# ska-sa/katsdpsigproc

Measured on AMD Instinct MI355X. Metric: visibility samples/s (baselines x channels) through full RFI flagger, higher is better.
Workload: dtype f32 amplitude / f64 deviations

## Files before the change

### katsdpsigproc_amd/csrc/ring_kernel.h

```cpp
#pragma once
#include "fused_common.h"

#ifndef RING_STOP
#define RING_STOP 0
#endif
#define RING_THREADS 512
#define RING_STRIP 8
#define RING_NSLOT 32
#ifndef RING_G
#define RING_G 4
#endif
#ifndef RING_PRIO
#define RING_PRIO 0
#endif
#ifndef RING_STAGGER
#define RING_STAGGER 0
#endif
#define RING_SLOT_BYTES 4096
#define RING_LIST_DOUBLES 256
#define RING_XCD_GROUP 8

struct RingLayout {
    static constexpr size_t RING_BYTES = (size_t)RING_NSLOT * RING_SLOT_BYTES;
    static constexpr size_t LIST_BYTES = sizeof(double) * RING_LIST_DOUBLES * RING_STRIP;
    static constexpr size_t CTRL_BYTES = 64;
    static constexpr size_t LDS_BYTES = RING_BYTES + LIST_BYTES + CTRL_BYTES;
};

#ifdef RING_TRACE
#define RING_TRACE_STRIPS 24
#define RING_TRACE_SLOTS 16
__device__ unsigned long long ring_trace_buf[256 * 8 * RING_TRACE_STRIPS * RING_TRACE_SLOTS];
#endif

#define RING_WORK_LIST 2
#define RING_WORK_DONE 10

__device__ __forceinline__ int ring_strip_of(int x, int t)
{
    return ((t / RING_XCD_GROUP) * 8 + x) * RING_XCD_GROUP + (t % RING_XCD_GROUP);
}

__device__ __forceinline__ int ring_take(unsigned *work, int x, int n_strips, int t0)
{
    for (int k = 0; k < 8; k++) {
        const int xx = (x + k) & 7;
        const int t = t0 + (int)atomicAdd(&work[RING_WORK_LIST + xx], 1u);
        const int s = ring_strip_of(xx, t);
        if (s < n_strips) return s;
    }
    return -1;
}

__device__ __forceinline__ float ring_from_next(float v, float edge, int lane)
{
    const float r = __shfl_down(v, 1, 64);
    return lane == 63 ? edge : r;
}
__device__ __forceinline__ float ring_from_prev(float v, float edge, int lane)
{
    const float r = __shfl_up(v, 1, 64);
    return lane == 0 ? edge : r;
}

template <int WIDTH>
__global__ __launch_bounds__(RING_THREADS) void flagger_ring_kernel(const FusedParams p)
{
    constexpr int R = 64, W = WIDTH, H = WIDTH / 2;
    constexpr int G = RING_G, NSLOT = RING_NSLOT, STEPS = 64, NCHUNK = STEPS / G;
    constexpr int K = NSLOT / G;
    constexpr int PER_CHUNK = G / 2;
    static_assert(W % 2 == 1 && W <= 13 && 2 * H <= G * 3, "merging median only");
    typedef __attribute__((address_space(3))) void lds_void;
    extern __shared__ __attribute__((aligned(16))) char lds[];
    const int tid = threadIdx.x, lane = tid & 63;
    const int wave = __builtin_amdgcn_readfirstlane(tid >> 6);
    const int C = p.channels;
    double *list = (double *)(lds + RingLayout::RING_BYTES) + wave * RING_LIST_DOUBLES;
    int *ctrl = (int *)(lds + RingLayout::RING_BYTES + RingLayout::LIST_BYTES);
    const unsigned lds_base = (unsigned)(size_t)(lds_void *)lds;

    const int q = wave & 3, par = wave >> 2;
    const int rl = lane >> 2;
    const int chunk16 = (lane & 3) ^ ((rl >> 2) & 3);
    const size_t row_bytes = (size_t)p.vis_stride * 8;
    const unsigned lane_off = (unsigned)((size_t)(16 * q + rl) * 64 * row_bytes + (size_t)chunk16 * 16);
    const int pp = wave >> 1, hh = wave & 1;
    const int l16 = lane & 15;
    const unsigned rd_off = (lane >> 4) * 1024 + l16 * 64 + ((pp ^ ((l16 >> 2) & 3)) * 16) + 8 * hh;
    typedef const __attribute__((address_space(3))) char lds_cchar;
    typedef const __attribute__((address_space(3))) unsigned long long lds_cu64;
    lds_cchar *lds3 = (lds_cchar *)(lds_void *)lds;

    unsigned long long run_src = 0;
    const unsigned long long rb2 = 2 * (unsigned long long)row_bytes;
    const unsigned piece_base = __builtin_amdgcn_readfirstlane(lds_base + q * 1024);
    auto issue = [&](int slot) {
        unsigned pb = piece_base;
        asm volatile("" : "+s"(pb));
        const unsigned dst = pb + (unsigned)(slot + par) * RING_SLOT_BYTES;
        unsigned keep;
        asm volatile("s_mov_b32 %0, m0\n\ts_mov_b32 m0, %3\n\ts_nop 0\n\t"
                     "global_load_lds_dwordx4 %1, %2\n\ts_mov_b32 m0, %0"
                     : "=&s"(keep) : "v"(lane_off), "s"(run_src), "s"(dst) : "memory");
        run_src += rb2;
    };
    auto strip_base = [&](int strip) -> const char * {
        return (const char *)p.vis + (size_t)strip * (RING_STRIP * 8);
    };

    const int xcd = blockIdx.x & 7;
    const int per_list = (int)gridDim.x >> 3;
    const int t0 = p.n_static * per_list;
    auto static_strip = [&](int k) { return ring_strip_of(xcd, k * per_list + ((int)blockIdx.x >> 3)); };
    if (tid == 0) {
        int s0 = 0 < p.n_static ? static_strip(0) : ring_take(p.work, xcd, p.n_strips, t0);
        int s1 = -1;
        if (s0 >= 0) s1 = 1 < p.n_static ? static_strip(1) : ring_take(p.work, xcd, p.n_strips, t0);
        ctrl[0] = s0;
        ctrl[1] = s1;
    }
    __syncthreads();
    int cur = __builtin_amdgcn_readfirstlane(ctrl[0]), nxt = __builtin_amdgcn_readfirstlane(ctrl[1]);
    int k_strip = 0;
    auto finish = [&]() {
        if (tid == 0 && atomicAdd(&p.work[RING_WORK_DONE], 1u) == gridDim.x - 1u) {
#pragma unroll
            for (int k = RING_WORK_LIST; k <= RING_WORK_DONE; k++) p.work[k] = 0;
        }
    };
    if (cur < 0) {
        finish();
        return;
    }
#if RING_STAGGER > 0
    if ((blockIdx.x >> 3) & 1) {
#pragma unroll
        for (int i = 0; i < RING_STAGGER; i++) __builtin_amdgcn_s_sleep(127);
    }
#endif
    auto start_of = [&](int strip) -> unsigned long long {
        const unsigned long long a = (unsigned long long)strip_base(strip) + (unsigned long long)par * row_bytes;
        return ((unsigned long long)(unsigned)__builtin_amdgcn_readfirstlane((unsigned)(a >> 32)) << 32) |
               (unsigned long long)(unsigned)__builtin_amdgcn_readfirstlane((unsigned)a);
    };
    run_src = start_of(cur);
#pragma unroll
    for (int j = 0; j < NSLOT; j += 2) issue(j);
    float2 zz[2][G];
    {
        constexpr int AH0 = (K - 1) * PER_CHUNK;
        __builtin_amdgcn_s_waitcnt(0x0070 | (AH0 & 15) | ((AH0 >> 4) << 14));
        __syncthreads();
#pragma unroll
        for (int g = 0; g < G; g++) {
            const unsigned long long w = *(lds_cu64 *)(lds3 + rd_off + g * RING_SLOT_BYTES);
            zz[0][g] = make_float2(__uint_as_float((unsigned)w), __uint_as_float((unsigned)(w >> 32)));
        }
    }
    const float nanv = __builtin_nanf("");
    const float2 *visf = (const float2 *)p.vis;

#if RING_PRIO == 1
    if (wave >= 4) __builtin_amdgcn_s_setprio(1);
#endif
    int mad_hint = -1;
    const int lane_id = lane;
#ifdef RING_TRACE
    int trace_it = 0;
#define RING_STAMP(i)                                                                              \
    do {                                                                                           \
        if (lane_id == 0 && trace_it < RING_TRACE_STRIPS && blockIdx.x < 256)                      \
            ring_trace_buf[((blockIdx.x * 8 + wave) * RING_TRACE_STRIPS + trace_it) * RING_TRACE_SLOTS + (i)] =   \
                __builtin_amdgcn_s_memtime();                                                      \
    } while (0)
#else
#define RING_STAMP(i) do { } while (0)
#endif
    for (;;) {
        int lane = lane_id;
        asm volatile("" : "+v"(lane));
        const int bl = cur * RING_STRIP + wave;
        const bool more = nxt >= 0;
        const unsigned long long start_nxt = start_of(more ? nxt : cur);
        auto fetch = [&](int c) -> float {
            const bool inside = c >= 0 && c < C;
            const int cc = inside ? c : 0;
            const float2 v = visf[(size_t)cc * p.vis_stride + bl];
            float a = ksp_abs_c64(v.x, v.y);
            return inside ? a : nanv;
        };
        RING_STAMP(0);
#ifdef RING_TRACE
        unsigned long long wait_dma = 0, wait_bar = 0;
        if (lane_id == 0 && trace_it < RING_TRACE_STRIPS && blockIdx.x < 256)
            ring_trace_buf[((blockIdx.x * 8 + wave) * RING_TRACE_STRIPS + trace_it) * RING_TRACE_SLOTS + 4] = __builtin_amdgcn_s_memrealtime();
#endif
        float amp[STEPS];
        unsigned umax = 0;
        auto load_chunk = [&](auto c_) {
            constexpr int c = decltype(c_)::value;
            constexpr int AH = (K - 2) * PER_CHUNK;
#ifdef RING_TRACE
            unsigned long long w0;
            asm volatile("s_memtime %0\n\ts_waitcnt lgkmcnt(0)" : "=s"(w0));
#endif
            if (more || (c + K - 1) * G + G <= STEPS)
                __builtin_amdgcn_s_waitcnt(0x0070 | (AH & 15) | ((AH >> 4) << 14));
            else
                __builtin_amdgcn_s_waitcnt(0x0070);
#ifdef RING_TRACE
            unsigned long long w1;
            asm volatile("s_memtime %0\n\ts_waitcnt lgkmcnt(0)" : "=s"(w1));
#endif
#ifndef RING_NOSYNC
            __syncthreads();
#endif
#ifdef RING_TRACE
            unsigned long long w2;
            asm volatile("s_memtime %0\n\ts_waitcnt lgkmcnt(0)" : "=s"(w2));
            wait_dma += w1 - w0;
            wait_bar += w2 - w1;
#endif
            ksp_static_for<G / 2>([&](auto u_) {
                constexpr int j = c * G + 2 * decltype(u_)::value + NSLOT;
                if constexpr (j < STEPS) {
                    issue(j % NSLOT);
                } else if (more) {
                    if constexpr (j == STEPS) run_src = start_nxt;
                    issue(j % NSLOT);
                }
            });
            if (c + 1 < NCHUNK || more) {
                unsigned ro = rd_off + (((c + 1) * G) % NSLOT) * RING_SLOT_BYTES;
                asm volatile("" : "+v"(ro));
#pragma unroll
                for (int g = 0; g < G; g++) {
                    const unsigned long long w = *(lds_cu64 *)(lds3 + ro + g * RING_SLOT_BYTES);
                    zz[(c + 1) & 1][g] = make_float2(__uint_as_float((unsigned)w), __uint_as_float((unsigned)(w >> 32)));
                }
            }
#if RING_PRIO == 2
            if ((c + (wave >> 2)) & 1)
                __builtin_amdgcn_s_setprio(1);
            else
                __builtin_amdgcn_s_setprio(0);
#endif
            const float2 (&z)[G] = zz[c & 1];
            unsigned key = ~0u;
#pragma unroll
            for (int g = 0; g < G; g++) key &= ksp_abs_range_key(z[g].x, z[g].y);
#pragma unroll
            for (int g = 0; g < G; g += 2)
                ksp_abs_c64_inrange_x2(z[g].x, z[g].y, z[g + 1].x, z[g + 1].y, amp[c * G + g],
                                       amp[c * G + g + 1]);
            if (ksp_any((key & KSP_ABS_RANGE_BIT) == 0)) {
#pragma unroll
                for (int g = 0; g < G; g++) {
                    amp[c * G + g] = ksp_abs_c64(z[g].x, z[g].y);
                    umax = max(umax, __float_as_uint(amp[c * G + g]));
                }
            }
        };

        float dev[R];
        float dmax;
        unsigned ex_a = 0, ex_b = 0;
        int tiny = 0;
        auto note_exact = [&](unsigned &acc, float x, float m, float d) {
            unsigned t;
            asm("v_min_u32 %1, %2, %3\n\tv_or_b32 %1, 0x7fffff, %1\n\t"
                "v_cmp_ge_f32 vcc, %1, |%4|\n\tv_addc_co_u32 %0, vcc, %0, %0, vcc"
                : "+v"(acc), "=&v"(t)
                : "v"(__float_as_uint(x)), "v"(__float_as_uint(m)), "v"(d)
                : "vcc");
        };
#if RING_STOP == 1
        dmax = 0.f;
        ksp_static_for<NCHUNK>([&](auto c_) {
            load_chunk(c_);
            constexpr int c = decltype(c_)::value;
#pragma unroll
            for (int g = 0; g < G; g++) {
                dev[c * G + g] = amp[c * G + g];
                dmax += amp[c * G + g];
            }
        });
#else
        {
            MergeMedian<R, W> mm;
            mm.pinf = __builtin_inff();
            mm.ninf = -__builtin_inff();
            asm volatile("" : "+v"(mm.pinf), "+v"(mm.ninf));
            const float pinf = mm.pinf, ninf = mm.ninf;
            const bool first = lane == 0, last = lane == 63;
            dmax = ninf;
            float rh[H];
            auto X = [&](auto i_) -> float {
                constexpr int i = decltype(i_)::value;
                if constexpr (i < STEPS) {
                    if constexpr (i % G == 0) load_chunk(std::integral_constant<int, i / G>{});
                    return amp[i];
                } else {
                    if constexpr (i == STEPS) {
#pragma unroll
                        for (int k = 0; k < H; k++)
                            rh[k] = ring_from_next(amp[k], (k & 1) ? ninf : pinf, lane);
                    }
                    return rh[i - STEPS];
                }
            };
            constexpr int RV = R - H;
            constexpr int STAGES = (RV + W - 1) / W;
            using MM = MergeMedian<R, W>;
            float cur_b[W];
            ksp_static_for<W>([&](auto k_) { cur_b[decltype(k_)::value] = X(k_); });
            ksp_static_for<STAGES>([&](auto m_) {
                constexpr int m = decltype(m_)::value;
                float S[MM::S_SIZE];
                S[MM::off(W - 1)] = cur_b[W - 1];
                ksp_static_for<W - 1>([&](auto u_) {
                    constexpr int t = W - 2 - decltype(u_)::value;
                    mm.template insert<W - 1 - t>(&S[MM::off(t + 1)], cur_b[t], &S[MM::off(t)]);
                });
                float P[W], nxt_b[W];
                ksp_static_for<W>([&](auto t_) {
                    constexpr int t = decltype(t_)::value;
                    constexpr int jv = m * W + t;
                    if constexpr (jv < RV) {
                        constexpr int j = jv + H;
                        if constexpr (t >= 1) {
                            nxt_b[t - 1] = X(std::integral_constant<int, (m + 1) * W + t - 1>{});
                            if constexpr (t == 1)
                                P[0] = nxt_b[0];
                            else
                                mm.template insert<t - 1>(P, nxt_b[t - 1], P);
                        }
                        const float med = mm.template rank<W - t, t, H>(&S[MM::off(t)], P);
                        const float xc = (t + H < W) ? cur_b[t + H < W ? t + H : 0] : nxt_b[t + H >= W ? t + H - W : 0];
                        float d = xc - med;
                        constexpr bool right_odd = j + H >= R && ((j + H - R + 1) & 1);
                        if constexpr (right_odd) {
                            const float lo = mm.template rank<W - t, t, H - 1>(&S[MM::off(t)], P);
                            if (last) {
                                const double dd = (double)xc - ((double)lo + (double)med) * 0.5;
                                d = (float)dd;
                                tiny += (d == 0.0f && dd != 0.0);
                            }
                        }
                        asm volatile("" : "+v"(d));
                        if constexpr (jv < 32)
                            note_exact(ex_a, xc, med, d);
                        else
                            note_exact(ex_b, xc, med, d);
                        if constexpr (jv & 1)
                            asm("v_max3_f32 %0, %0, %1, %2" : "+v"(dmax) : "v"(dev[j - 1]), "v"(d));
                        else if constexpr (jv == RV - 1)
                            dmax = mm.vmax(dmax, d);
                        dev[j] = d;
                    }
                });
                if constexpr (m + 1 < STAGES) {
                    ksp_static_for<W>([&](auto k_) {
                        constexpr int k = decltype(k_)::value;
                        constexpr int i = (m + 1) * W + k;
                        constexpr bool have = (m * W + k + 1 < RV) && (k + 1 < W);
                        if constexpr (!have) {
                            if constexpr (i < R + H)
                                nxt_b[k] = X(std::integral_constant<int, i>{});
                            else
                                nxt_b[k] = pinf;
                        }
                    });
#pragma unroll
                    for (int k = 0; k < W; k++) cur_b[k] = nxt_b[k];
                }
            });
            if constexpr (H >= 1) {
                float L[H];
#pragma unroll
                for (int k = 0; k < H; k++)
                    L[k] = ring_from_prev(amp[STEPS - H + k], ((H - k) & 1) ? pinf : ninf, lane);
                constexpr auto soff = [](int j) { return j * H - j * (j - 1) / 2; };
                float SL[H * (H + 1) / 2];
                SL[soff(H - 1)] = L[H - 1];
                ksp_static_for<H - 1>([&](auto u_) {
                    constexpr int j = H - 2 - decltype(u_)::value;
                    mm.template insert<H - 1 - j>(&SL[soff(j + 1)], L[j], &SL[soff(j)]);
                });
                float PL[2 * H];
                PL[0] = amp[0];
                ksp_static_for<H>([&](auto k_) {
                    constexpr int k = decltype(k_)::value + 1;
                    mm.template insert<k>(PL, amp[k], PL);
                });
                ksp_static_for<H>([&](auto j_) {
                    constexpr int j = decltype(j_)::value;
                    if constexpr (j >= 1) mm.template insert<j + H>(PL, amp[j + H], PL);
                    const float med = mm.template rank<H - j, j + H + 1, H>(&SL[soff(j)], PL);
                    const float xc = amp[j];
                    float d = xc - med;
                    if constexpr ((H - j) & 1) {
                        const float lo = mm.template rank<H - j, j + H + 1, H - 1>(&SL[soff(j)], PL);
                        if (first) {
                            const double dd = (double)xc - ((double)lo + (double)med) * 0.5;
                            d = (float)dd;
                            tiny += (d == 0.0f && dd != 0.0);
                        }
                    }
                    note_exact(ex_b, xc, med, d);
                    dmax = mm.vmax(dmax, d);
                    dev[j] = d;
                });
            }
        }
#endif
        RING_STAMP(1);
#ifdef RING_TRACE
        if (lane_id == 0 && trace_it < RING_TRACE_STRIPS && blockIdx.x < 256) {
            ring_trace_buf[((blockIdx.x * 8 + wave) * RING_TRACE_STRIPS + trace_it) * RING_TRACE_SLOTS + 5] = wait_dma;
            ring_trace_buf[((blockIdx.x * 8 + wave) * RING_TRACE_STRIPS + trace_it) * RING_TRACE_SLOTS + 6] = wait_bar;
        }
#endif
        unsigned long long exact;
        {
            const unsigned ra = __builtin_bitreverse32(ex_a), rb = __builtin_bitreverse32(ex_b);
            exact = ((unsigned long long)ra << H) |
                    ((unsigned long long)(rb & ((1u << (32 - H)) - 1u)) << (H + 32)) |
                    (unsigned long long)(rb >> (32 - H));
            unsigned long long first_odd = 0, last_odd = 0;
#pragma unroll
            for (int j = 0; j < H; j++)
                if ((H - j) & 1) first_odd |= 1ull << j;
#pragma unroll
            for (int j = R - H; j < R; j++)
                if ((j + H - R + 1) & 1) last_odd |= 1ull << j;
            if (lane == 0) exact &= ~first_odd;
            if (lane == 63) exact &= ~last_odd;
        }
        if (ksp_any(umax >= 0x7f800000u)) {
            float a2[R + 2 * H];
            int c_first = lane * R - H;
            asm volatile("" : "+v"(c_first));
#pragma unroll
            for (int i = 0; i < R + 2 * H; i++) a2[i] = fetch(c_first + i);
            tiny = 0;
            median_phase_src<R, W>([&](int i) { return a2[i + H]; }, dev, dmax, &tiny);
            exact = 0;
        }
        const bool ticket = more && k_strip + 2 >= p.n_static;
        unsigned t_own = 0;
        if (tid == 0 && ticket) t_own = atomicAdd(&p.work[RING_WORK_LIST + xcd], 1u);

#if RING_STOP == 1 || RING_STOP == 2
        {
            float acc = dmax;
#pragma unroll
            for (int j = 0; j < R; j++) acc += dev[j];
            if (acc == 12345.678f && p.noise != nullptr) p.noise[bl] = acc;
        }
#else
        const double noise64 = mad_noise<R, W, RING_LIST_DOUBLES, true>(dev, lane, list, fetch, RING_STOP > 30 ? RING_STOP : 0,
#ifdef RING_TRACE
                                                                      (trace_it < RING_TRACE_STRIPS && blockIdx.x < 256)
                                                                          ? &ring_trace_buf[((blockIdx.x * 8 + wave) * RING_TRACE_STRIPS + trace_it) * RING_TRACE_SLOTS]
                                                                          : nullptr,
#else
                                                                      nullptr,
#endif
                                                                      exact, &mad_hint, tiny);
        if (lane == 0 && p.noise != nullptr) p.noise[bl] = (float)noise64;
        RING_STAMP(2);
#if RING_STOP == 3 || RING_STOP > 30
        if (noise64 == 12345.678 && p.noise != nullptr) p.noise[bl] = dmax;
#else
        const unsigned long long fl = threshold_flags<R, W>(p, dev, dmax, noise64, lane, C, fetch);
        write_flags(p, fl, lane * R, bl, C);
        RING_STAMP(3);
#endif
#endif

#ifdef RING_TRACE
        if (lane_id == 0 && trace_it < RING_TRACE_STRIPS && blockIdx.x < 256)
            ring_trace_buf[((blockIdx.x * 8 + wave) * RING_TRACE_STRIPS + trace_it) * RING_TRACE_SLOTS + 7] = (unsigned long long)cur + 1;
        trace_it++;
#endif
        if (!more) break;
        cur = nxt;
        if (!ticket) {
            nxt = static_strip(k_strip + 2);
#ifdef RING_END_SYNC
            __syncthreads();
#endif
        } else {
            if (tid == 0) {
                int take = ring_strip_of(xcd, t0 + (int)t_own);
                if (take >= p.n_strips) take = ring_take(p.work, (xcd + 1) & 7, p.n_strips, t0);
                ctrl[2] = take;
            }
            __syncthreads();
            nxt = __builtin_amdgcn_readfirstlane(ctrl[2]);
            __syncthreads();
        }
        k_strip++;
    }
    finish();
}

inline bool ring_supported(const FusedParams &p, int width)
{
    return p.channels == 4096 && width % 2 == 1 && width >= 3 && width <= 13 && !p.is_amplitude &&
           p.flags_mode == KSP_FLAGS_NONE && p.deviations == nullptr && p.work != nullptr &&
           p.baselines >= RING_STRIP && (p.vis_stride % 2) == 0 &&
           (p.threshold_kind != KSP_THRESHOLD_SUM || p.n_windows <= 4) &&
           (size_t)p.vis_stride * 8 * 4096 < 0x7fffff00ull;
}

template <int WIDTH>
inline int launch_ring(int device, hipStream_t s, const FusedParams &p_in, int n_cu, hipEvent_t ev0,
                       hipEvent_t ev1)
{
    FusedParams p = p_in;
    p.n_strips = p.baselines / RING_STRIP;
    auto kern = flagger_ring_kernel<WIDTH>;
    static std::atomic<bool> attr_set[64];
    if (device < 0 || device >= 64 || !attr_set[device].load(std::memory_order_acquire)) {
        KSP_CHECK(hipFuncSetAttribute((const void *)kern, hipFuncAttributeMaxDynamicSharedMemorySize,
                                      (int)RingLayout::LDS_BYTES));
        if (device >= 0 && device < 64) attr_set[device].store(true, std::memory_order_release);
    }
    const int grid = p.n_strips < n_cu ? p.n_strips : n_cu;
    p.n_static = 0;
    if (grid % 8 == 0 && p.n_strips / grid >= 3) {
        const int by_share = p.n_strips / grid - 2;
        const int by_range = (8 * (p.n_strips / 64)) / (grid / 8);
        p.n_static = by_share < by_range ? by_share : by_range;
    }
#ifndef RING_STATIC
    p.n_static = 0;
#endif
#ifdef RING_TRACE
    {
        void *tb = nullptr;
        KSP_CHECK(hipGetSymbolAddress(&tb, HIP_SYMBOL(ring_trace_buf)));
        KSP_CHECK(hipMemsetAsync(tb, 0, sizeof(ring_trace_buf), s));
    }
#endif
    if (ev0 != nullptr)
        hipExtLaunchKernelGGL(kern, dim3(grid), dim3(RING_THREADS), RingLayout::LDS_BYTES, s, ev0, ev1,
                              0, p);
    else
        hipLaunchKernelGGL(kern, dim3(grid), dim3(RING_THREADS), RingLayout::LDS_BYTES, s, p);
    KSP_LAUNCH_CHECK();
#ifdef RING_TRACE
    if (const char *path = getenv("KSP_RING_TRACE")) {
        KSP_CHECK(hipStreamSynchronize(s));
        const size_t n = sizeof(ring_trace_buf);
        void *host = malloc(n);
        KSP_CHECK(hipMemcpyFromSymbol(host, HIP_SYMBOL(ring_trace_buf), n));
        FILE *f = fopen(path, "wb");
        if (f != nullptr) {
            fwrite(host, 1, n, f);
            fclose(f);
        }
        free(host);
    }
#endif
    return 0;
}
```

Before: 351.5 billion.

## Deepen LDS read/convert pipeline and specialize streaming loop on more-strips flag

The amplitude computation now runs one chunk ahead: each load step reads chunk c+2 from LDS and converts chunk c+1, and the first chunk of the next strip is carried across strips in amp_nxt. The DMA wait threshold is relaxed by one chunk to match. The whole median stream is instantiated twice, once for a compile-time 'more' and once without, so runtime branches inside become constexpr. The aim is to hide LDS latency and abs conversion behind median work, at the cost of more live registers and a larger code footprint.

```diff
diff --git a/katsdpsigproc_amd/csrc/ring_kernel.h b/katsdpsigproc_amd/csrc/ring_kernel.h
--- a/katsdpsigproc_amd/csrc/ring_kernel.h
+++ b/katsdpsigproc_amd/csrc/ring_kernel.h
@@ -148,15 +148,40 @@
 #pragma unroll
     for (int j = 0; j < NSLOT; j += 2) issue(j);
     float2 zz[2][G];
+    auto read_chunk = [&](int chunk, float2 (&z)[G]) {
+        unsigned ro = rd_off + ((chunk * G) % NSLOT) * RING_SLOT_BYTES;
+        asm volatile("" : "+v"(ro));
+#pragma unroll
+        for (int g = 0; g < G; g++) {
+            const unsigned long long w = *(lds_cu64 *)(lds3 + ro + g * RING_SLOT_BYTES);
+            z[g] = make_float2(__uint_as_float((unsigned)w), __uint_as_float((unsigned)(w >> 32)));
+        }
+    };
+    auto convert_chunk = [&](const float2 (&z)[G], float *a, unsigned &um) {
+        static_assert(G == 4, "the pin below names four results");
+        unsigned key = ~0u;
+#pragma unroll
+        for (int g = 0; g < G; g++) key &= ksp_abs_range_key(z[g].x, z[g].y);
+#pragma unroll
+        for (int g = 0; g < G; g += 2)
+            ksp_abs_c64_inrange_x2(z[g].x, z[g].y, z[g + 1].x, z[g + 1].y, a[g], a[g + 1]);
+        asm volatile("" : "+v"(a[0]), "+v"(a[1]), "+v"(a[2]), "+v"(a[3]));
+        if (ksp_any((key & KSP_ABS_RANGE_BIT) == 0)) {
+#pragma unroll
+            for (int g = 0; g < G; g++) {
+                a[g] = ksp_abs_c64(z[g].x, z[g].y);
+                um = max(um, __float_as_uint(a[g]));
+            }
+        }
+    };
+    float amp_nxt[G];
+    unsigned umax_nxt = 0;
     {
         constexpr int AH0 = (K - 1) * PER_CHUNK;
         __builtin_amdgcn_s_waitcnt(0x0070 | (AH0 & 15) | ((AH0 >> 4) << 14));
         __syncthreads();
-#pragma unroll
-        for (int g = 0; g < G; g++) {
-            const unsigned long long w = *(lds_cu64 *)(lds3 + rd_off + g * RING_SLOT_BYTES);
-            zz[0][g] = make_float2(__uint_as_float((unsigned)w), __uint_as_float((unsigned)(w >> 32)));
-        }
+        read_chunk(0, zz[0]);
+        convert_chunk(zz[0], amp_nxt, umax_nxt);
     }
     const float nanv = __builtin_nanf("");
     const float2 *visf = (const float2 *)p.vis;
@@ -197,15 +222,19 @@
             ring_trace_buf[((blockIdx.x * 8 + wave) * RING_TRACE_STRIPS + trace_it) * RING_TRACE_SLOTS + 4] = __builtin_amdgcn_s_memrealtime();
 #endif
         float amp[STEPS];
-        unsigned umax = 0;
-        auto load_chunk = [&](auto c_) {
+        unsigned umax = umax_nxt;
+        umax_nxt = 0;
+#pragma unroll
+        for (int g = 0; g < G; g++) amp[g] = amp_nxt[g];
+        auto load_chunk = [&](auto more_, auto c_) {
+            constexpr bool MORE = decltype(more_)::value;
             constexpr int c = decltype(c_)::value;
-            constexpr int AH = (K - 2) * PER_CHUNK;
+            constexpr int AH = (K - 3) * PER_CHUNK;
 #ifdef RING_TRACE
             unsigned long long w0;
             asm volatile("s_memtime %0\n\ts_waitcnt lgkmcnt(0)" : "=s"(w0));
 #endif
-            if (more || (c + K - 1) * G + G <= STEPS)
+            if constexpr (MORE || (c + K - 1) * G + G <= STEPS)
                 __builtin_amdgcn_s_waitcnt(0x0070 | (AH & 15) | ((AH >> 4) << 14));
             else
                 __builtin_amdgcn_s_waitcnt(0x0070);
@@ -226,41 +255,23 @@
                 constexpr int j = c * G + 2 * decltype(u_)::value + NSLOT;
                 if constexpr (j < STEPS) {
                     issue(j % NSLOT);
-                } else if (more) {
+                } else if constexpr (MORE) {
                     if constexpr (j == STEPS) run_src = start_nxt;
                     issue(j % NSLOT);
                 }
             });
-            if (c + 1 < NCHUNK || more) {
-                unsigned ro = rd_off + (((c + 1) * G) % NSLOT) * RING_SLOT_BYTES;
-                asm volatile("" : "+v"(ro));
-#pragma unroll
-                for (int g = 0; g < G; g++) {
-                    const unsigned long long w = *(lds_cu64 *)(lds3 + ro + g * RING_SLOT_BYTES);
-                    zz[(c + 1) & 1][g] = make_float2(__uint_as_float((unsigned)w), __uint_as_float((unsigned)(w >> 32)));
-                }
-            }
+            if constexpr (c == 0) read_chunk(1, zz[1]);
+            if constexpr (c + 2 < NCHUNK || (MORE && c + 2 == NCHUNK)) read_chunk(c + 2, zz[c & 1]);
 #if RING_PRIO == 2
             if ((c + (wave >> 2)) & 1)
                 __builtin_amdgcn_s_setprio(1);
             else
                 __builtin_amdgcn_s_setprio(0);
 #endif
-            const float2 (&z)[G] = zz[c & 1];
-            unsigned key = ~0u;
-#pragma unroll
-            for (int g = 0; g < G; g++) key &= ksp_abs_range_key(z[g].x, z[g].y);
-#pragma unroll
-            for (int g = 0; g < G; g += 2)
-                ksp_abs_c64_inrange_x2(z[g].x, z[g].y, z[g + 1].x, z[g + 1].y, amp[c * G + g],
-                                       amp[c * G + g + 1]);
-            if (ksp_any((key & KSP_ABS_RANGE_BIT) == 0)) {
-#pragma unroll
-                for (int g = 0; g < G; g++) {
-                    amp[c * G + g] = ksp_abs_c64(z[g].x, z[g].y);
-                    umax = max(umax, __float_as_uint(amp[c * G + g]));
-                }
-            }
+            if constexpr (c + 1 < NCHUNK)
+                convert_chunk(zz[(c + 1) & 1], &amp[(c + 1) * G], umax);
+            else if constexpr (MORE)
+                convert_chunk(zz[(c + 1) & 1], amp_nxt, umax_nxt);
         };
 
         float dev[R];
@@ -275,19 +286,19 @@
                 : "v"(__float_as_uint(x)), "v"(__float_as_uint(m)), "v"(d)
                 : "vcc");
         };
+        auto stream = [&](auto more_) __attribute__((always_inline)) {
 #if RING_STOP == 1
-        dmax = 0.f;
-        ksp_static_for<NCHUNK>([&](auto c_) {
-            load_chunk(c_);
-            constexpr int c = decltype(c_)::value;
-#pragma unroll
-            for (int g = 0; g < G; g++) {
-                dev[c * G + g] = amp[c * G + g];
-                dmax += amp[c * G + g];
-            }
-        });
+            dmax = 0.f;
+            ksp_static_for<NCHUNK>([&](auto c_) {
+                load_chunk(more_, c_);
+                constexpr int c = decltype(c_)::value;
+#pragma unroll
+                for (int g = 0; g < G; g++) {
+                    dev[c * G + g] = amp[c * G + g];
+                    dmax += amp[c * G + g];
+                }
+            });
 #else
-        {
             MergeMedian<R, W> mm;
             mm.pinf = __builtin_inff();
             mm.ninf = -__builtin_inff();
@@ -299,7 +310,7 @@
             auto X = [&](auto i_) -> float {
                 constexpr int i = decltype(i_)::value;
                 if constexpr (i < STEPS) {
-                    if constexpr (i % G == 0) load_chunk(std::integral_constant<int, i / G>{});
+                    if constexpr (i % G == 0) load_chunk(more_, std::integral_constant<int, i / G>{});
                     return amp[i];
                 } else {
                     if constexpr (i == STEPS) {
@@ -413,8 +424,12 @@
                     dev[j] = d;
                 });
             }
-        }
-#endif
+#endif
+        };
+        if (more)
+            stream(std::true_type{});
+        else
+            stream(std::false_type{});
         RING_STAMP(1);
 #ifdef RING_TRACE
         if (lane_id == 0 && trace_it < RING_TRACE_STRIPS && blockIdx.x < 256) {
```

New measurement: 363.1 billion, median of 6. 1.03x the previous value.
